# NoSuchThingAsRandom/EpidemicSimulator

Hardware: AMD Instinct MI355X
Metric: citizen-timesteps/sec (higher is better)
Workload: dtype u32 citizen word; u32 uniform vs ceil(q*2^32) (reference: f64 uniform; tolerance 2^-32 per draw); 1 GPU; uk64m: 64000000 citizens, 290000 Output Areas, 10 seeds, steps 1..667 of 5000, interventions on; seed=1592598545

## Files before the change

### epidemicsimulator_amd/csrc/esim_device.h

```cpp
#pragma once
#include <stdint.h>

#define CW_TE_SHIFT    19u
#define CW_BUS_EXPOSED (1u << 18)
#define CW_FLAGS       0xFFu
#define CW_VAX_SHIFT   11u
#define CW_VAX_MASK    (0x7Fu << CW_VAX_SHIFT)
#define CW_KEEP        (CW_FLAGS | CW_VAX_MASK)
#define CW_VAX_NONE    0xFFFFFFFFu
#define CW_PLAN_SKIP   (1u << 10)
#define CW_VAX_REL(w)  ((((w) >> CW_VAX_SHIFT) & 0x7Fu) ? 127u - (((w) >> CW_VAX_SHIFT) & 0x7Fu) : CW_VAX_NONE)
#define CW_VAX_FIELD(j) ((127u - (j)) << CW_VAX_SHIFT)
#define CW_TE(w)       ((w) >> CW_TE_SHIFT)
#define CW_MAKE(te, rest) (((te) << CW_TE_SHIFT) | (rest))
#define TE_SUSCEPTIBLE 0x1FFFu
#define TE_VACCINATED  0x1FFEu
#define TE_RECOVERED   0x1FFDu
#define TE_BIAS        512u
#define TE_SLOTS       8192u
#define ESIM_MAX_STEP  7600u

#define FL_USES_PT        0x01u
#define FL_MASK_COMPLIANT 0x02u
#define FL_SAME_AREA      0x04u
// ... 184 lines not shown
    uint32_t *prof_buf;
#endif
    uint32_t xf_n;
    const uint32_t *bld_area;
    uint32_t n_areas;
};

#define XA_HEADER 8u
#define XB_HEADER 8u
#define FREE_MAX 96u
#define HKEY_EMPTY 0xFFFFFFFFFFFFFFFFull
#define PLAN_W 4096u
#define XV_HEADER 8u
#define XS_CAP_MAX (1u << 20)
#define HOT_STRIDE 32u
#define SUBQ 64u
#define HOT_NEWEXP 0u
#define HOT_UNITS 64u
#define HOT_BIGPAIRS 128u
#define HOT_BIG 129u
#define HOT_PREV_NEWEXP 257u
#define HOT_RESET 257u
#define HOT_LOST 321u
#define HOT_COUNT 322u
#define RAISE(ctrl, code, where) do { (ctrl)->error = (uint32_t)(-(code)); (ctrl)->err_where = (where); } while (0)
enum { ERR_AT_BIG_LIST = 2, ERR_AT_ITEM_CHECK = 6, ERR_AT_ROUTE_ITEM = 7, ERR_AT_BIGPAIRS = 10, ERR_AT_SCHOOL = 11 };
#define UNIT_NOOP 0xFFFFFFFFu
#ifndef LOST_CAP
#define LOST_CAP 8192u
#endif
#define CHUNK_BUS_STEPS 32u
#define PAIR_K(per_wave, nbus) ((per_wave) * ((nbus) > 8u ? ((nbus) + 3u) / 4u : 2u))
#define COUNT_GRID 256u
#define EXP_ROWS 32u
#ifndef UNIT_INLINE
#define UNIT_INLINE 1024u
#endif
#ifndef UNIT_PAIRS
#define UNIT_PAIRS 1024u
#endif
#define CHUNK_ROUTE_MAX 2048u
```

### epidemicsimulator_amd/csrc/esim_host_ctx.h

```cpp
namespace {

thread_local std::string g_create_error;

struct Timing {
    bool phase = false, kernel = false;
    uint32_t stride = 16;
    hipEvent_t ev[5] = { nullptr, nullptr, nullptr, nullptr, nullptr };
    double phase_s[3] = { 0, 0, 0 };
    std::vector<hipEvent_t> kev; size_t kev_used = 0;
    hipEvent_t cev[2] = { nullptr, nullptr }; double chunk_ms = 0; uint64_t chunk_steps = 0, chunk_count = 0;
    std::vector<hipEvent_t> pkev; size_t pkev_used = 0; uint64_t pipe_steps = 0;
    hipEvent_t sev[2] = { nullptr, nullptr }; double small_ms = 0; uint64_t small_steps = 0;
    bool kdetail = false;
    std::vector<hipEvent_t> kdev; std::vector<int> kd_kind; size_t kd_used = 0;
    double kd_ms[ESIM_CK_N] = { 0 }; uint64_t kd_calls[ESIM_CK_N] = { 0 };
    bool host_trace = false;
    std::vector<std::pair<const char *, double>> ht;

    static void make_pair(hipEvent_t (&e)[2]) { if (!e[0]) { (void)hipEventCreate(&e[0]); (void)hipEventCreate(&e[1]); } }
    void clear()
    {
        phase_s[0] = phase_s[1] = phase_s[2] = 0;
        kev_used = 0; pkev_used = 0; pipe_steps = 0;
        small_ms = 0; small_steps = 0; chunk_ms = 0; chunk_steps = 0; chunk_count = 0;
// ... 61 lines not shown
    uint32_t step = 0;
    esim_params P;
    Ctrl h;
    uint32_t *words = nullptr, *hist = nullptr, *log_off = nullptr, *exp_step = nullptr;
    esim_step_result *records = nullptr;
    uint32_t *log = nullptr; size_t log_cap = 0;
    uint32_t last_chunk_pairs = 0; bool quiet = false, repair_armed = false, elig_seen = false;
    uint64_t vax_chunk_steps = 0, vax_chunk_cuts = 0, vax_chunk_repairs = 0;
};

struct Seam { uint32_t step = 0, rate = 0; uint64_t seed = 0; };

struct DrawSeam { uint32_t step = 0; bool twice = false, two_capacities = false; uint64_t seed = 0; double chance = 0.0, mask_effectiveness = 0.0; };

struct Tuning {
    uint32_t grid_citizens = 1, grid_infected = 1, grid_expose = 1;
    uint32_t grid_chunk = 1024;
    bool grid_chunk_env = false;
    bool pipeline = true;
    bool time_parallel = true;
    bool vax_chunks = true;
    bool vax_repair = true;
    bool vax_repair_always = false;
    uint32_t tiny_pairs = 2048;
    uint32_t small_grid = 64, small_mult = 4;
    uint32_t draw_mult = 4, units_mult = 4;
    uint32_t small_max = 128;
};

struct esim_ctx_impl {
    esim_params P;
    Dev d;
    bool uploaded = false;
    hipStream_t stream = nullptr;
    std::string err;
    std::vector<uint32_t> init_state;
    std::vector<uint32_t> init_log;
    size_t cnt_bytes = 0;
    uint32_t *cnt_base = nullptr;
    uint32_t n_routes = 0;
    size_t xa_n = 0, xb_n = 0, xf_n = 0;
    uint64_t pop_hash = 0;
    uint64_t pop_hash_head = 0;
    uint32_t cap_steps = 0;
    uint32_t *area_cnt = nullptr;
    uint32_t *arrival = nullptr;
// ... 243 lines not shown
```

### epidemicsimulator_amd/csrc/esim_host_run.h

```cpp
namespace {

int enqueue_begin(esim_ctx_impl *c, bool time_kernel)
{
    Dev &d = c->d;
    if (c->tm.phase) HIP_TRY(c, hipEventRecord(c->tm.ev[0], c->stream));
    if (time_kernel) HIP_TRY(c, hipEventRecord(c->tm.kev[c->tm.kev_used + 0], c->stream));
    hipLaunchKernelGGL(k_infected, dim3(c->tune.grid_infected), dim3(TPB), 0, c->stream, d);
    if (d.n_shards > 1) {
        const uint32_t n = (uint32_t)std::max<size_t>(XA_HEADER, std::max(d.n_shared_bld, d.n_shared_room));
        hipLaunchKernelGGL(k_pack_a, dim3(grid_for(n, TPB, 1u << 20)), dim3(TPB), 0, c->stream, d);
    }
    if (c->tm.phase) HIP_TRY(c, hipEventRecord(c->tm.ev[1], c->stream));
    return ESIM_OK;
}

int enqueue_exposures(esim_ctx_impl *c)
{
    Dev &d = c->d;
    if (d.n_shards > 1) {
        const uint32_t n = (uint32_t)std::max<size_t>(XA_HEADER, std::max(d.n_shared_bld, d.n_shared_room));
        hipLaunchKernelGGL(k_unpack_a, dim3(grid_for(n, TPB, 1u << 20)), dim3(TPB), 0, c->stream, d);
    }
    hipLaunchKernelGGL(k_expose, dim3(c->tune.grid_expose), dim3(TPB), 0, c->stream, d);
    if (d.n_shards > 1) hipLaunchKernelGGL(k_pack_b, dim3(VACC_WINDOW / TPB), dim3(TPB), 0, c->stream, d);
// ... 113 lines not shown
bool tiny_chunk(const esim_ctx_impl *c) { return c->tune.tiny_pairs && c->last_chunk_pairs <= c->tune.tiny_pairs && c->d.world == 1u && c->d.n_shards == 1u; }
bool small_chunk(const esim_ctx_impl *c) { return c->tune.small_grid && c->last_chunk_pairs < 4096u && c->tune.grid_chunk > c->tune.small_grid && !c->tune.grid_chunk_env; }

struct ChunkPass {
    esim_ctx_impl *c;
    uint32_t limit_t;
    bool kd;
    uint32_t n_ahead() const { return (uint32_t)c->xf_n; }
    void mark(int kind) const { if (kd) kd_mark(c, kind); }
    void future(uint32_t n) const { mark(ESIM_CK_FUTURE); hipLaunchKernelGGL(k_future, dim3(1), dim3(FIN_TPB), 0, c->stream, c->d, n, limit_t); }
    void decide(uint32_t n, int parallel, int vax_in_census) const { mark(ESIM_CK_DECIDE); hipLaunchKernelGGL(k_decide, dim3(1), dim3(64), 0, c->stream, c->d, n, limit_t, parallel, vax_in_census); }
    void vax_plan(int sharded) const { mark(ESIM_CK_VAX); hipLaunchKernelGGL(k_chunk_vax<false>, dim3(FREE_MAX + (sharded ? 0u : 1u)), dim3(FIN_TPB), 0, c->stream, c->d, n_ahead(), limit_t, sharded); }
    void lost() const { mark(ESIM_CK_VAX_REPAIR); hipLaunchKernelGGL(k_chunk_lost, dim3(1), dim3(FIN_TPB), 0, c->stream, c->d); }
    void vax_repair(int sharded) const { hipLaunchKernelGGL(k_chunk_vax<true>, dim3(FREE_MAX), dim3(FIN_TPB), 0, c->stream, c->d, n_ahead(), limit_t, sharded); }
    void front(bool few) const
    {
        const Tuning &t = c->tune;
        const uint32_t g = few ? t.small_grid : t.grid_chunk, g_draw = g * (few ? t.small_mult : t.draw_mult), g_units = g * (few ? t.small_mult : t.units_mult);
        mark(ESIM_CK_MARKS); hipLaunchKernelGGL(k_chunk_marks, dim3(g), dim3(TPB), 0, c->stream, c->d);
        mark(ESIM_CK_FOLD); hipLaunchKernelGGL(k_chunk_fold, dim3(g), dim3(TPB), 0, c->stream, c->d);
        mark(ESIM_CK_DRAW); hipLaunchKernelGGL(k_chunk_draw, dim3(g_draw), dim3(TPB), 0, c->stream, c->d, g * (TPB / 64u));
        mark(ESIM_CK_UNITS); hipLaunchKernelGGL(k_chunk_units, dim3(g_units), dim3(TPB), 0, c->stream, c->d);
    }
    void count() const { mark(ESIM_CK_COUNT); hipLaunchKernelGGL(k_chunk_count, dim3(COUNT_GRID), dim3(TPB), 0, c->stream, c->d); }
    void scatter() const { mark(ESIM_CK_SCATTER); hipLaunchKernelGGL(k_chunk_scatter, dim3(COUNT_GRID), dim3(TPB), 0, c->stream, c->d); }
    void books(int alone, int then_next) const { mark(ESIM_CK_BOOKS); hipLaunchKernelGGL(k_chunk_books, dim3(1), dim3(FIN_TPB), 0, c->stream, c->d, alone, then_next, n_ahead(), limit_t); }
    void vax_final() const { mark(ESIM_CK_VAX_FINAL); hipLaunchKernelGGL(k_chunk_vax_final, dim3(FREE_MAX), dim3(TPB), 0, c->stream, c->d); }
};

void enqueue_parallel_chunk(esim_ctx_impl *c, int then_next, uint32_t limit_t)
{
    const ChunkPass p{ c, limit_t, true };
    const bool alone = c->last_chunk_pairs < 1024u;
    p.front(small_chunk(c));
    if (!alone) p.count();
    p.books(alone ? 1 : 0, then_next);
    if (!alone) p.scatter();
    p.mark(ESIM_CK_N);
}

void enqueue_vax_chunk(esim_ctx_impl *c, uint32_t limit_t)
{
    const ChunkPass p{ c, limit_t, true };
    const Tuning &t = c->tune;
    const bool quiet = c->quiet && c->d.world == 1u;
    p.vax_plan(0);
    p.decide(p.n_ahead(), 1, 0);
    if (!quiet) {
        p.front(small_chunk(c));
        if (c->d.world == 1u && t.vax_repair && (c->repair_armed || t.vax_repair_always)) { p.lost(); p.vax_repair(0); }
    }
    p.count();
    p.books(0, 0);
    if (!quiet) p.scatter();
    p.vax_final();
    p.mark(ESIM_CK_N);
}

void enqueue_free_burst(esim_ctx_impl *c, uint32_t bursts, uint32_t limit_t)
{
    const ChunkPass p{ c, limit_t, true };
    if (tiny_chunk(c)) {
        for (uint32_t g = 0; g < bursts; ++g) {
            p.mark(ESIM_CK_TINY);
            hipLaunchKernelGGL(k_chunk_tiny, dim3(1), dim3(FIN_TPB), 0, c->stream, c->d, g == 0u ? 1 : 0, g + 1u < bursts ? 1 : 0, p.n_ahead(), limit_t);
        }
        p.mark(ESIM_CK_N);
        return;
    }
    p.future(p.n_ahead());
    p.decide(p.n_ahead(), 1, 0);
    for (uint32_t g = 0; g < bursts; ++g) enqueue_parallel_chunk(c, g + 1u < bursts ? 1 : 0, limit_t);
}

int run_chunk(esim_ctx_impl *c, uint32_t n_ahead, uint32_t *executed, Ctrl *state_before)
{
    Dev &d = c->d; Timing &t = c->tm;
// ... 233 lines not shown
```

### epidemicsimulator_amd/csrc/esim_host_shard.h

```cpp
namespace {

#define RCCL_ENTRIES(X) X(GetUniqueId) X(CommInitRank) X(CommDestroy) X(CommAbort) X(Send) X(Recv) X(GroupStart) X(GroupEnd) X(AllReduce) X(GetErrorString)
struct RcclApi {
#define X(f) decltype(&nccl##f) f = nullptr;
    RCCL_ENTRIES(X)
#undef X
    bool ok = false;
};

RcclApi &rccl()
{
    static RcclApi api;
    static bool tried = false;
    if (tried) return api;
    tried = true;
    void *h = nullptr;
    for (const char *name : { "librccl.so", "librccl.so.1" }) if ((h = dlopen(name, RTLD_NOW | RTLD_NOLOAD))) break;
    if (!h) for (const char *name : { "librccl.so.1", "librccl.so", "/opt/rocm/lib/librccl.so.1" }) if ((h = dlopen(name, RTLD_NOW | RTLD_GLOBAL))) break;
    if (!h) return api;
    api.ok = true;
#define X(f) if (!(api.f = (decltype(api.f))dlsym(h, "nccl" #f))) api.ok = false;
    RCCL_ENTRIES(X)
#undef X
    return api;
// ... 226 lines not shown
    int rc;
    p.future(n_ahead);
    if (vax) {
        hipLaunchKernelGGL(k_vax_live<false>, dim3(PLAN_W / TPB, FREE_MAX), dim3(TPB), 0, c->stream, d, n_ahead, limit_t);
        if ((rc = exchange_buf(c, 3, d.xv, xv_n))) return rc;
        p.vax_plan(1);
    }
    const size_t seg = 1u + 3u * (size_t)d.xs_cap;
    for (uint32_t r = 0; r < d.world; ++r) HIP_TRY(c, hipMemsetAsync(d.xs_out + (size_t)r * seg, 0, sizeof(uint32_t), c->stream));
    hipLaunchKernelGGL(k_shared_pack, dim3(256), dim3(TPB), 0, c->stream, d, n_ahead, limit_t);
    if ((rc = exchange_alltoall(c, 4, d.xs_out, d.xs, seg))) return rc;
    hipLaunchKernelGGL(k_shard_prep, dim3(1), dim3(128), 0, c->stream, d, n_ahead, limit_t);
    if ((rc = exchange(c, 2))) return rc;
    p.decide(n_ahead, 1, 1);
    p.front(false);
    if (vax && c->tune.vax_repair && (c->repair_armed || c->tune.vax_repair_always)) {
        p.lost();
        if ((rc = exchange_buf(c, 10, d.xl, FREE_MAX + 2u))) return rc;
        hipLaunchKernelGGL(k_lost_global, dim3(1), dim3(64), 0, c->stream, d);
        hipLaunchKernelGGL(k_vax_live<true>, dim3(PLAN_W / TPB, FREE_MAX), dim3(TPB), 0, c->stream, d, n_ahead, limit_t);
        if ((rc = exchange_buf(c, 3, d.xv, xv_n))) return rc;
        p.vax_repair(1);
    }
    p.count();
    if (vax && (rc = exchange_buf(c, 5, d.xc, FREE_MAX + 2u))) return rc;
    p.books(0, 0);
    p.scatter();
    p.vax_final();
    HIP_TRY(c, hipGetLastError());
    return ESIM_OK;
}

int run_coupled_steps(esim_ctx_impl *c, uint32_t n, bool ex)
{
    int rc;
    for (uint32_t s = 0; s < n; ++s) {
        const bool tk = want_kernel_timing(c);
        if ((rc = enqueue_begin(c, tk))) return rc;
        if (ex && (rc = exchange(c, 0))) return rc;
        if ((rc = enqueue_exposures(c))) return rc;
        if (ex && (rc = exchange(c, 1))) return rc;
        if ((rc = enqueue_finish(c, tk))) return rc;
        if ((s & 255u) == 255u && (rc = wait_stream(c))) return rc;
    }
    c->comm.step_steps += n;
    return ESIM_OK;
}

}

// ... 70 lines not shown
```

### epidemicsimulator_amd/csrc/esim_host_upload.h

```cpp
namespace {

struct UploadHost {
    const esim_population *pop;
    uint32_t N, B, R, n_global;
    bool sharded;
    std::vector<uint8_t> fl;
    std::vector<uint32_t> room_fixed;
    std::vector<uint32_t> route_off, riders, route_of;
    uint32_t n_routes = 0, max_route = 0, n_big_routes = 0;
    bool any_big = false;
    std::vector<uint32_t> res_off, res_idx, wrk_off, wrk_idx, room_off, room_idx;
    bool home_sorted = true;
};

int upload_validate(esim_ctx_impl *c, UploadHost &u)
{
    const esim_population *pop = u.pop; const uint32_t N = u.N, B = u.B, R = u.R;
    if (!pop->home_building || !pop->work_building || !pop->room || !pop->flags || !pop->building_area || !pop->building_type)
        return fail(c, ESIM_EINVAL, "esim_upload_population: a required array is NULL");
    if (R && !pop->room_building) return fail(c, ESIM_EINVAL, "esim_upload_population: room_building is NULL");
    if (pop->n_seeds && !pop->seeds) return fail(c, ESIM_EINVAL, "esim_upload_population: seeds is NULL");
    u.n_global = pop->n_citizens_global ? pop->n_citizens_global : N;
    if ((uint64_t)pop->citizen_id_base + N > u.n_global) return fail(c, ESIM_EINVAL, "esim_upload_population: shard range exceeds n_citizens_global");
    u.sharded = u.n_global != N || pop->n_shared_buildings || pop->n_shared_rooms;
// ... 184 lines not shown
        d.n_sch = n_sch;
        if ((rc = dev_upload(c, &d.sch_of_bld, sch_of.data(), sch_of.size()))) return rc;
    }
    {
        std::vector<uint4> w4(N ? N : 1);
        for (uint32_t i = 0; i < N; ++i) w4[i] = make_uint4(pop->home_building[i], pop->work_building[i], u.room_fixed[i], u.route_of[i]);
        if ((rc = dev_upload(c, &d.where4, w4.data(), w4.size()))) return rc;
        std::vector<BldRec> b8(B ? B : 1);
        for (uint32_t b = 0; b < B; ++b) b8[b] = BldRec{ u.res_off[b], u.res_off[b + 1], u.wrk_off[b], u.wrk_off[b + 1], (uint32_t)pop->building_type[b], ovf_off[b], ovf_off[b + 1], 0u };
        if ((rc = dev_upload(c, &d.bld8, b8.data(), b8.size()))) return rc;
        if ((rc = dev_alloc_fill(c, &d.sch_diff, (size_t)(d.n_sch ? d.n_sch : 1) * SD_REPL * 2u * FREE_MAX))) return rc;
    }
    d.ovf_room_base = ovf_off.back();
    d.ovf_n = d.ovf_room_base + u.room_off.back() + 1u;
    if ((rc = dev_alloc_fill(c, &d.ovf, (size_t)d.ovf_n))) return rc;
    d.n_wrk_idx = (uint32_t)u.wrk_idx.size(); d.n_room_idx = (uint32_t)u.room_idx.size();
    d.big_qcap = d.items_cap / SUBQ;
    if ((rc = dev_alloc_fill(c, &d.big_list, (size_t)d.big_qcap * SUBQ * 3u))) return rc;
    if ((rc = dev_alloc_fill(c, &d.used_pref, CHUNK_WAVES_MAX + 1u))) return rc;
    if ((rc = dev_alloc_fill(c, &d.pair_cnt, 16384u)) || (rc = dev_alloc_fill(c, &d.used_cnt, 16384u))) return rc;
    if ((rc = dev_alloc_fill(c, &d.hot, (size_t)HOT_COUNT * HOT_STRIDE))) return rc;
    d.newexp_cap = N / SUBQ + 1u;
    if ((rc = dev_alloc_fill(c, &d.newexp, (size_t)d.newexp_cap * SUBQ))) return rc;
    if ((rc = dev_alloc_fill(c, &d.cursor, (size_t)EXP_ROWS * FREE_MAX))) return rc;
    return ESIM_OK;
}

int upload_step_tables(esim_ctx_impl *c, const UploadHost &u)
{
    const uint32_t N = u.N, B = u.B, R = u.R;
    Dev &d = c->d; int rc;
    const size_t per_parity = (size_t)B + R + u.n_routes;
    for (int p = 0; p < (int)MARK_SLOTS; ++p) {
        uint32_t *base = c->cnt_base + p * per_parity;
        d.cnt_bld[p] = base; d.cnt_room[p] = base + B; d.route_flag[p] = base + B + R;
        if ((rc = dev_alloc(c, &d.touched_bld[p], B)) || (rc = dev_alloc(c, &d.touched_room[p], R))) return rc;
        if ((rc = dev_alloc(c, &d.touched_route[p], u.n_routes)) || (rc = dev_alloc(c, &d.touched_route_big[p], u.n_routes))) return rc;
    }
    if ((rc = dev_alloc(c, &d.vax_ev, (size_t)FREE_MAX * VACC_MAX_RATE))) return rc;
    if ((rc = dev_alloc_fill(c, &d.vax_cnt, FREE_MAX)) || (rc = dev_alloc_fill(c, &d.vax_now, FREE_MAX))) return rc;
    if ((rc = dev_alloc_fill(c, &d.vax_delta, 4u * (FREE_MAX + 2u)))) return rc;
    if ((rc = dev_alloc_fill(c, &d.lost_list, LOST_CAP))) return rc;
    if ((rc = dev_alloc_fill(c, &d.xf_adj, FREE_MAX + 2u))) return rc;
    if ((rc = dev_alloc(c, &d.hist, TE_SLOTS)) || (rc = dev_alloc(c, &d.log, (size_t)N + 1)) || (rc = dev_alloc(c, &d.log_off, TE_SLOTS + 1))) return rc;
    {
        const uint32_t *sd = nullptr;
        if ((rc = dev_upload(c, &sd, c->init_log.data(), c->init_log.size()))) return rc;
// ... 50 lines not shown
}

int upload_pinned(esim_ctx_impl *c, const UploadHost &u)
{
    if (!c->pin.ctrl) HIP_TRY(c, hipHostMalloc((void **)&c->pin.ctrl, sizeof(Ctrl), hipHostMallocDefault));
    if (!c->rs.stage) HIP_TRY(c, hipHostMalloc((void **)&c->rs.stage, sizeof(*c->rs.stage), hipHostMallocDefault));
    if (!c->rs.ev) HIP_TRY(c, hipEventCreateWithFlags(&c->rs.ev, hipEventDisableTiming));
    if (int rc = pinned_grow(c, &c->pin.rec, &c->pin.rec_n, (size_t)c->cap_steps + 1)) return rc;
    return pinned_grow(c, &c->pin.area, &c->pin.area_n, (size_t)u.pop->n_areas * 5u);
}

void upload_tuning(esim_ctx_impl *c, const UploadHost &u)
{
    Tuning &t = c->tune;
    t.grid_citizens = grid_for(u.N, TPB, 2048);
    t.grid_infected = 1024;
    t.grid_expose = 1024;
    if (const char *e = std::getenv("ESIM_GRID_INFECTED")) t.grid_infected = (uint32_t)std::max(1, std::atoi(e));
    const char *gc = std::getenv("ESIM_GRID_CHUNK");
    t.grid_chunk_env = gc != nullptr;
    if (gc) t.grid_chunk = (uint32_t)std::min((int)(CHUNK_WAVES_MAX * 64u / TPB), std::max(16, std::atoi(gc) / 16 * 16));
    if (std::getenv("ESIM_TRACE_HOST")) c->tm.host_trace = true;
    if (const char *e = std::getenv("ESIM_VAX_REPAIR")) { t.vax_repair = std::atoi(e) != 0; t.vax_repair_always = std::atoi(e) >= 2; }
    if (const char *e = std::getenv("ESIM_TINY_PAIRS")) t.tiny_pairs = (uint32_t)std::max(0, std::atoi(e));
    if (const char *e = std::getenv("ESIM_SMALL_GRID")) t.small_grid = (uint32_t)std::max(0, std::atoi(e) / 16 * 16);
    if (const char *e = std::getenv("ESIM_SMALL_MULT")) t.small_mult = (uint32_t)std::min(16, std::max(1, std::atoi(e)));
    if (const char *e = std::getenv("ESIM_DRAW_MULT")) t.draw_mult = (uint32_t)std::min(4, std::max(1, std::atoi(e)));
    if (const char *e = std::getenv("ESIM_UNITS_MULT")) t.units_mult = (uint32_t)std::min(16, std::max(1, std::atoi(e)));
    if (const char *e = std::getenv("ESIM_GRID_EXPOSE")) t.grid_expose = (uint32_t)std::max(1, std::atoi(e));
}

}

extern "C" int esim_upload_population(esim_ctx *ctx, const esim_population *pop)
{
    esim_ctx_impl *c = CTX(ctx);
    if (!c || !pop) return fail(c, ESIM_EINVAL, "esim_upload_population: null argument");
    HIP_TRY(c, hipSetDevice(c->P.device));
    UploadHost u;
    u.pop = pop; u.N = pop->n_citizens; u.B = pop->n_buildings; u.R = pop->n_rooms;
    int rc;
    if ((rc = upload_validate(c, u))) return rc;
    c->pop_hash = population_hash(pop, &c->pop_hash_head);
    upload_routes(u);
    upload_member_lists(u);
    c->init_state.resize(u.N);
// ... 164 lines not shown
```

### epidemicsimulator_amd/csrc/esim_kernels_books.h

```cpp
#pragma once
#include "esim_kernels_common.h"
#include "esim_kernels_plan.h"
#include "esim_kernels_marks.h"
__global__ __launch_bounds__(TPB) void k_chunk_count(Dev d)
{
    Ctrl *ctrl = d.ctrl;
    if (!ctrl->chunk_parallel || ctrl->chunk_ok == 0u) return;
    const uint32_t tid = blockIdx.x * TPB + threadIdx.x, r = tid & (SUBQ - 1u), step = (gridDim.x * TPB) / SUBQ;
    const uint32_t n_new = newexp_len(d, HOT_NEWEXP, r);
    const uint32_t *list = newexp_list(d, r);
    const uint32_t t0 = ctrl->chunk_t0;
    __shared__ uint32_t e_cnt[2u * FREE_MAX];
    __shared__ uint32_t s_cut;
    if (threadIdx.x < 2u * FREE_MAX) e_cnt[threadIdx.x] = 0u;
    if (threadIdx.x == 0) s_cut = 0xFFFFFFFFu;
    __syncthreads();
    for (uint32_t i = tid / SUBQ; i < n_new; i += step) {
        if (list[i] >= d.n) continue;
        const uint32_t w = d.cit[list[i]];
        const uint32_t j = CW_TE(w) - TE_BIAS - t0;
        if (j < FREE_MAX) atomicAdd(&e_cnt[2u * j + ((w & CW_BUS_EXPOSED) ? 1u : 0u)], 1u);
        if ((w & CW_BUS_EXPOSED) && CW_VAX_REL(w) != CW_VAX_NONE) { atomicMin(&s_cut, j); if (d.world > 1u) d.xc[j] = 1u; }
    }
    __syncthreads();
    if (threadIdx.x < 2u * FREE_MAX && e_cnt[threadIdx.x]) atomicAdd(&d.exp_part[(size_t)(blockIdx.x % EXP_ROWS) * 2u * FREE_MAX + threadIdx.x], e_cnt[threadIdx.x]);
    if (threadIdx.x == 0 && s_cut != 0xFFFFFFFFu) atomicMin(&ctrl->chunk_cut, s_cut);
    if (!ctrl->vax_chunk) return;
    __shared__ int dl[4][FREE_MAX + 2];
    for (uint32_t i = threadIdx.x; i < 4u * (FREE_MAX + 2u); i += TPB) (&dl[0][0])[i] = 0;
    __syncthreads();
    const uint32_t n = ctrl->chunk_ok;
    for (uint32_t j = blockIdx.x; j < n; j += gridDim.x) {
        const uint32_t cnt = d.vax_cnt[j];
        for (uint32_t i = threadIdx.x; i < cnt; i += TPB) {
            const uint32_t w = d.cit[d.vax_ev[(size_t)j * VACC_MAX_RATE + i]], te = CW_TE(w);
            if (CW_VAX_REL(w) != j) continue;
            atomicAdd(&dl[3][j + 1u], 1);
            if (te == TE_SUSCEPTIBLE || (te < TE_RECOVERED && te - TE_BIAS - t0 < n && te - TE_BIAS - t0 > j)) { atomicSub(&dl[0][j + 1u], 1); continue; }
            const int e_last = (int)te - (int)TE_BIAS + (int)d.exposed_time - (int)t0, i_last = e_last + 1 + (int)d.infected_time;
            const int lo = (int)j + 1;
            if (lo <= e_last) { atomicSub(&dl[1][lo], 1); atomicAdd(&dl[1][min(e_last, (int)n - 1) + 1], 1); }
            const int ilo = max(lo, e_last + 1);
            if (ilo <= i_last && ilo < (int)n) { atomicSub(&dl[2][ilo], 1); atomicAdd(&dl[2][min(i_last, (int)n - 1) + 1], 1); }
        }
    }
    __syncthreads();
    for (uint32_t i = threadIdx.x; i < 4u * (FREE_MAX + 2u); i += TPB) { const int v = (&dl[0][0])[i]; if (v) atomicAdd(&d.vax_delta[i], (uint32_t)v); }
}

__global__ __launch_bounds__(TPB) void k_chunk_scatter(Dev d)
{
    Ctrl *ctrl = d.ctrl;
    if (ctrl->chunk_done == 0u) return;
    const uint32_t t0 = ctrl->prev_t0;
    const uint32_t n_items = min(ctrl->prev_n_items, d.items_cap);
    {
        const uint32_t tid = blockIdx.x * TPB + threadIdx.x, r = tid & (SUBQ - 1u), step = (gridDim.x * TPB) / SUBQ;
        const uint32_t n_new = newexp_len(d, HOT_PREV_NEWEXP, r);
        const uint32_t *list = newexp_list(d, r);
        const uint32_t n_eff = ctrl->prev_n_eff;
        for (uint32_t i = tid / SUBQ; i < n_new; i += step) {
            const uint32_t m = list[i];
            if (m >= d.n) continue;
            const uint32_t te = CW_TE(d.cit[m]);
            if (te - TE_BIAS - t0 < n_eff) d.log[d.log_off[te] + atomicAdd(&d.cursor[(blockIdx.x % EXP_ROWS) * FREE_MAX + te - TE_BIAS - t0], 1u)] = m;
            else {
                const bool again = ctrl->prev_cut && te - TE_BIAS - t0 == n_eff && (d.cit[m] & CW_BUS_EXPOSED);
                atomicOr(&d.cit[m], (TE_SUSCEPTIBLE << CW_TE_SHIFT) | (again ? CW_PLAN_SKIP : 0u));
                atomicAnd(&d.cit[m], ~CW_BUS_EXPOSED);
            }
        }
    }
    const uint32_t per_wave = ctrl->prev_per_wave, n_mw = per_wave ? n_items / per_wave : 0u;
    const uint32_t tid = blockIdx.x * TPB + threadIdx.x, nth = gridDim.x * TPB;
    for (uint32_t i = tid; i < n_mw * per_wave; i += nth) {
        const uint32_t w = i / per_wave, k = i - w * per_wave;
        if (k >= d.used_cnt[w]) continue;
        const uint32_t h = d.hitems[i];
        if (h >= d.hcap) continue;
        const uint32_t state = d.slot_state[h];
        if (state > ITEM_RECS && d.item_rec[i].id < d.n_bld + d.n_room)
            for (uint32_t j = 0; j < FREE_MAX; ++j) d.vec[(size_t)h * FREE_MAX + j] = 0u;
        d.hkey[h] = HKEY_EMPTY;
        if (state) d.slot_state[h] = 0u;
    }
}

__global__ __launch_bounds__(TPB) void k_chunk_vax_final(Dev d)
{
    Ctrl *ctrl = d.ctrl;
    if (!ctrl->prev_vax) return;
    const uint32_t n_eff = ctrl->prev_n_eff;
    const uint32_t n = ctrl->prev_planned;
    for (uint32_t j = blockIdx.x; j < n; j += gridDim.x) {
        const uint32_t cnt = d.vax_cnt[j];
        for (uint32_t i = threadIdx.x; i < cnt; i += TPB) {
            const uint32_t c = d.vax_ev[(size_t)j * VACC_MAX_RATE + i];
            const uint32_t w = d.cit[c];
            if (CW_VAX_REL(w) != j) continue;
            if (j < n_eff) {
                const uint32_t te = CW_TE(w);
                if (te < TE_RECOVERED) atomicSub(&d.hist[te], 1u);
                d.cit[c] = CW_MAKE(TE_VACCINATED, w & (CW_BUS_EXPOSED | CW_FLAGS));
            } else atomicAnd(&d.cit[c], ~CW_VAX_MASK);
        }
    }
}

// ... 86 lines not shown
        ctrl->n_vaccinated = V0 + cum[3][n_eff];
        if (vax) ctrl->elig_count = elig0 - cum[4][n_eff];
        ctrl->log_len = run0 + (P[top0 + (int)n_eff] - P[top0]);
        ctrl->t = t0 + n_eff; ctrl->steps_done = t0 + n_eff - 1u;
        if (n_eff < n_cut) ctrl->finished = 1u;
        else if (n_cut < n) ctrl->vax_cuts += 1u;
        ctrl->prev_cut = (n_eff == n_cut && n_cut < n && !(vax && ctrl->repair_ran)) ? 1u : 0u;
        if (n_eff) {
            ctrl->lockdown = d.dec[n_eff].lockdown; ctrl->mask = d.dec[n_eff].mask;
            ctrl->at_work = d.dec[n_eff - 1u].at_work; ctrl->bus_dir = d.dec[n_eff - 1u].bus_dir;
        }
        const uint32_t keep = marks_left ? ((t0 + n - 1u) & (MARK_SLOTS - 1u)) : MARK_SLOTS;
        for (uint32_t z = 0; z < MARK_SLOTS; ++z)
            if (z != keep) { ctrl->n_touched_bld[z] = 0u; ctrl->n_touched_room[z] = 0u; ctrl->n_touched_route[z] = 0u; ctrl->n_touched_route_big[z] = 0u; }
    }
    return n_eff;
}

__global__ __launch_bounds__(FIN_TPB) void k_batch_finish(Dev d, uint32_t t0, uint32_t n)
{
    batch_finish_body(d, t0, n);
}

struct BooksShared { uint32_t e_cnt[2 * FREE_MAX]; uint32_t lo_s[FREE_MAX], cur_s[FREE_MAX]; uint32_t win[BF_WIN]; uint32_t wtmp[FIN_TPB / 64]; };
__device__ __forceinline__ void books_body(const Dev &d, int fused, int do_next, uint32_t max_ahead, uint32_t limit_t, BooksShared &bs)
{
    uint32_t *e_cnt = bs.e_cnt, *lo_s = bs.lo_s, *cur_s = bs.cur_s, *win = bs.win, *wtmp = bs.wtmp;
    Ctrl *ctrl = d.ctrl;
    const uint32_t tid = threadIdx.x;
    const uint32_t pb0 = PROF_NOW();
    if (!ctrl->chunk_parallel || ctrl->chunk_ok == 0u) {
        if (tid == 0) {
            ctrl->chunk_done = 0u;
            ctrl->prev_vax = ld(&ctrl->vax_chunk); ctrl->prev_n_eff = 0u; ctrl->prev_planned = ld(&ctrl->vax_planned); ctrl->vax_chunk = 0u;
        }
        return;
    }
    const uint32_t t0 = ctrl->chunk_t0, n = ctrl->chunk_ok;
    const uint32_t n_items = min(ld(&ctrl->n_items), d.items_cap);
    if (tid < 2u * FREE_MAX) e_cnt[tid] = 0u;
    if (tid < FREE_MAX) cur_s[tid] = 0u;
    __syncthreads();
    const uint32_t r = tid & (SUBQ - 1u);
    const uint32_t n_new = newexp_len(d, HOT_NEWEXP, r);
    const uint32_t *list = newexp_list(d, r);
    if (fused) {
        for (uint32_t i = tid / SUBQ; i < n_new; i += FIN_TPB / SUBQ) {
            if (list[i] >= d.n) continue;
            const uint32_t w = d.cit[list[i]];
            const uint32_t j = CW_TE(w) - TE_BIAS - t0;
            if (j < FREE_MAX) atomicAdd(&e_cnt[2u * j + ((w & CW_BUS_EXPOSED) ? 1u : 0u)], 1u);
        }
    } else if (tid < 2u * n) {
        uint32_t a = 0u, run = 0u;
        uint32_t v[EXP_ROWS];
#pragma unroll
        for (uint32_t p = 0; p < EXP_ROWS; ++p) v[p] = d.exp_part[(size_t)p * 2u * FREE_MAX + tid];
#pragma unroll
        for (uint32_t p = 0; p < EXP_ROWS; ++p) {
            d.exp_part[(size_t)p * 2u * FREE_MAX + tid] = 0u;
            a += v[p];
            if (!(tid & 1u)) d.cursor[p * FREE_MAX + (tid >> 1)] = run;
            run += v[p] + __shfl_xor(v[p], 1, 64);
        }
        e_cnt[tid] = a;
    }
    __syncthreads();
    const uint32_t pb1 = PROF_NOW();
    const bool vax = ld(&ctrl->vax_chunk) != 0u;
    const uint32_t n_eff = batch_finish_body(d, t0, n, e_cnt, lo_s, vax, false);
    const uint32_t pb2 = PROF_NOW();
    if (!fused) {
        if (tid < SUBQ) d.hot[(HOT_PREV_NEWEXP + tid) * HOT_STRIDE] = n_new;
        if (tid == 0) { ctrl->prev_t0 = t0; ctrl->prev_n_items = n_items; ctrl->prev_per_wave = ld(&ctrl->items_per_wave);
                        ctrl->prev_n = n; ctrl->prev_n_eff = n_eff; ctrl->prev_vax = vax ? 1u : 0u; ctrl->prev_planned = ld(&ctrl->vax_planned); ctrl->vax_chunk = 0u; }
    }
    if (tid == 0) ctrl->chunk_done = 1u;
    if (tid < 64u) {
        uint32_t a = ld(&d.hot[(HOT_NEWEXP + tid) * HOT_STRIDE]), b = ld(&d.hot[(HOT_UNITS + tid) * HOT_STRIDE]);
        for (int o = 32; o > 0; o >>= 1) { a += __shfl_xor(a, o, 64); b += __shfl_xor(b, o, 64); }
        if (tid == 0) { ctrl->n_newexp = a; ctrl->n_units = b; ctrl->n_route_pairs_big = ld(&d.hot[HOT_BIGPAIRS * HOT_STRIDE]); }
    }
    __syncthreads();
    if (fused) {
        for (uint32_t i = tid / SUBQ; i < n_new; i += FIN_TPB / SUBQ) {
            const uint32_t m = list[i];
            if (m >= d.n) continue;
            const uint32_t j = CW_TE(d.cit[m]) - TE_BIAS - t0;
            if (j < FREE_MAX) d.log[lo_s[j] + atomicAdd(&cur_s[j], 1u)] = m;
        }
        const uint32_t per_wave = ld(&ctrl->items_per_wave), n_mw = per_wave ? n_items / per_wave : 0u;
        for (uint32_t w0 = tid; w0 < n_mw; w0 += 4u * FIN_TPB) {
            uint32_t used[4], h[4][4];
#pragma unroll
            for (int a = 0; a < 4; ++a) { const uint32_t w = w0 + (uint32_t)a * FIN_TPB; used[a] = w < n_mw ? d.used_cnt[w] : 0u; }
#pragma unroll
            for (int a = 0; a < 4; ++a)
#pragma unroll
                for (int k = 0; k < 4; ++k) h[a][k] = (uint32_t)k < used[a] ? d.hitems[(w0 + (uint32_t)a * FIN_TPB) * per_wave + (uint32_t)k] : ITEM_UNUSED;
            uint32_t st[4][4];
#pragma unroll
            for (int a = 0; a < 4; ++a)
#pragma unroll
                for (int k = 0; k < 4; ++k) st[a][k] = h[a][k] < d.hcap ? d.slot_state[h[a][k]] : 0u;
#pragma unroll
            for (int a = 0; a < 4; ++a) {
                const uint32_t base = (w0 + (uint32_t)a * FIN_TPB) * per_wave;
// ... 7 lines not shown
                    if (state) d.slot_state[hs] = 0u;
                }
                for (uint32_t k = 4u; k < used[a]; ++k) {
                    const uint32_t hs = d.hitems[base + k];
                    if (hs >= d.hcap) continue;
                    const uint32_t state = d.slot_state[hs];
                    if (state > ITEM_RECS && d.item_rec[base + k].id < d.n_bld + d.n_room)
                        for (uint32_t j = 0; j < FREE_MAX; ++j) d.vec[(size_t)hs * FREE_MAX + j] = 0u;
                    d.hkey[hs] = HKEY_EMPTY;
                    if (state) d.slot_state[hs] = 0u;
                }
            }
        }
    }
    const uint32_t pb3 = PROF_NOW();
    if (do_next) {
        __syncthreads();
        future_body(d, max_ahead, limit_t, win, wtmp);
        __syncthreads();
        const uint32_t pb4 = PROF_NOW();
        if (tid < 64u) decide_body(d, max_ahead, limit_t, 1);
        BOOKS_PROF(d, 4, pb4 - pb3);
    }
    BOOKS_PROF(d, 0, pb1 - pb0); BOOKS_PROF(d, 1, pb2 - pb1); BOOKS_PROF(d, 2, pb3 - pb2); BOOKS_PROF(d, 3, PROF_NOW() - pb3);
    (void)pb0; (void)pb1; (void)pb2; (void)pb3;
}

__global__ __launch_bounds__(FIN_TPB) void k_chunk_books(Dev d, int fused, int do_next, uint32_t max_ahead, uint32_t limit_t)
{
    __shared__ BooksShared bs;
    books_body(d, fused, do_next, max_ahead, limit_t, bs);
}
```

Before: 57760 billion citizen-timesteps/s.

## Fuse chunk books and log scatter into one wide tail kernel

Adds a tail path, on by default when world==1, that moves hash-map cleanup into extra blocks of the count kernel. Books then runs as block 0 of a new multi-block tail kernel whose other blocks do the new-exposure log scatter for the current chunk, so the scatter no longer waits for the next chunk's scatter launch. Each block recomputes the prefix offsets from exp_part, and a last-block ticket zeroes exp_part. This removes a serial kernel launch and lets the single-block books work overlap the parallel scatter. In exchange it adds duplicated prefix work, ticket atomics and a second cursor array, and risks ordering bugs in the cut/skip logic.

```diff
diff --git a/epidemicsimulator_amd/csrc/esim_device.h b/epidemicsimulator_amd/csrc/esim_device.h
--- a/epidemicsimulator_amd/csrc/esim_device.h
+++ b/epidemicsimulator_amd/csrc/esim_device.h
@@ -230,7 +230,13 @@
 #define HOT_PREV_NEWEXP 257u
 #define HOT_RESET 257u
 #define HOT_LOST 321u
-#define HOT_COUNT 322u
+#define HOT_TAIL_RAN 322u
+#define HOT_TAIL_T0 323u
+#define HOT_TAIL_N 324u
+#define HOT_TAIL_VAX 325u
+#define HOT_TAIL_READERS 326u
+#define HOT_COUNT 327u
+#define HOT(d, i) ((d).hot[(i) * HOT_STRIDE])
 #define RAISE(ctrl, code, where) do { (ctrl)->error = (uint32_t)(-(code)); (ctrl)->err_where = (where); } while (0)
 enum { ERR_AT_BIG_LIST = 2, ERR_AT_ITEM_CHECK = 6, ERR_AT_ROUTE_ITEM = 7, ERR_AT_BIGPAIRS = 10, ERR_AT_SCHOOL = 11 };
 #define UNIT_NOOP 0xFFFFFFFFu
@@ -240,6 +246,7 @@
 #define CHUNK_BUS_STEPS 32u
 #define PAIR_K(per_wave, nbus) ((per_wave) * ((nbus) > 8u ? ((nbus) + 3u) / 4u : 2u))
 #define COUNT_GRID 256u
+#define CLEAN_GRID 1024u
 #define EXP_ROWS 32u
 #ifndef UNIT_INLINE
 #define UNIT_INLINE 1024u
diff --git a/epidemicsimulator_amd/csrc/esim_host_ctx.h b/epidemicsimulator_amd/csrc/esim_host_ctx.h
--- a/epidemicsimulator_amd/csrc/esim_host_ctx.h
+++ b/epidemicsimulator_amd/csrc/esim_host_ctx.h
@@ -107,6 +107,7 @@
     bool vax_chunks = true;
     bool vax_repair = true;
     bool vax_repair_always = false;
+    uint32_t chunk_tail = 2;
     uint32_t tiny_pairs = 2048;
     uint32_t small_grid = 64, small_mult = 4;
     uint32_t draw_mult = 4, units_mult = 4;
diff --git a/epidemicsimulator_amd/csrc/esim_host_run.h b/epidemicsimulator_amd/csrc/esim_host_run.h
--- a/epidemicsimulator_amd/csrc/esim_host_run.h
+++ b/epidemicsimulator_amd/csrc/esim_host_run.h
@@ -159,8 +159,15 @@
         mark(ESIM_CK_DRAW); hipLaunchKernelGGL(k_chunk_draw, dim3(g_draw), dim3(TPB), 0, c->stream, c->d, g * (TPB / 64u));
         mark(ESIM_CK_UNITS); hipLaunchKernelGGL(k_chunk_units, dim3(g_units), dim3(TPB), 0, c->stream, c->d);
     }
-    void count() const { mark(ESIM_CK_COUNT); hipLaunchKernelGGL(k_chunk_count, dim3(COUNT_GRID), dim3(TPB), 0, c->stream, c->d); }
-    void scatter() const { mark(ESIM_CK_SCATTER); hipLaunchKernelGGL(k_chunk_scatter, dim3(COUNT_GRID), dim3(TPB), 0, c->stream, c->d); }
+    void count(int tail) const { mark(ESIM_CK_COUNT); hipLaunchKernelGGL(k_chunk_count, dim3(COUNT_GRID + (tail ? CLEAN_GRID : 0u)), dim3(TPB), 0, c->stream, c->d, tail); }
+    void scatter(int clean) const { mark(ESIM_CK_SCATTER); hipLaunchKernelGGL(k_chunk_scatter, dim3(COUNT_GRID), dim3(TPB), 0, c->stream, c->d, clean); }
+    void tail(int then_next) const { mark(ESIM_CK_BOOKS); hipLaunchKernelGGL(k_chunk_tail, dim3(TAIL_GRID), dim3(FIN_TPB), 0, c->stream, c->d, then_next, n_ahead(), limit_t); }
+    void wide_tail(int then_next) const
+    {
+        const uint32_t form = c->d.world == 1u ? c->tune.chunk_tail : 0u;
+        if (form == 2u) { count(1); tail(then_next); }
+        else { count(form ? 1 : 0); books(0, then_next); scatter(form ? 0 : 1); }
+    }
     void books(int alone, int then_next) const { mark(ESIM_CK_BOOKS); hipLaunchKernelGGL(k_chunk_books, dim3(1), dim3(FIN_TPB), 0, c->stream, c->d, alone, then_next, n_ahead(), limit_t); }
     void vax_final() const { mark(ESIM_CK_VAX_FINAL); hipLaunchKernelGGL(k_chunk_vax_final, dim3(FREE_MAX), dim3(TPB), 0, c->stream, c->d); }
 };
@@ -170,9 +177,8 @@
     const ChunkPass p{ c, limit_t, true };
     const bool alone = c->last_chunk_pairs < 1024u;
     p.front(small_chunk(c));
-    if (!alone) p.count();
-    p.books(alone ? 1 : 0, then_next);
-    if (!alone) p.scatter();
+    if (alone) p.books(1, then_next);
+    else p.wide_tail(then_next);
     p.mark(ESIM_CK_N);
 }
 
@@ -187,9 +193,8 @@
         p.front(small_chunk(c));
         if (c->d.world == 1u && t.vax_repair && (c->repair_armed || t.vax_repair_always)) { p.lost(); p.vax_repair(0); }
     }
-    p.count();
-    p.books(0, 0);
-    if (!quiet) p.scatter();
+    if (quiet) { p.count(0); p.books(0, 0); }
+    else p.wide_tail(0);
     p.vax_final();
     p.mark(ESIM_CK_N);
 }
diff --git a/epidemicsimulator_amd/csrc/esim_host_shard.h b/epidemicsimulator_amd/csrc/esim_host_shard.h
--- a/epidemicsimulator_amd/csrc/esim_host_shard.h
+++ b/epidemicsimulator_amd/csrc/esim_host_shard.h
@@ -272,10 +272,10 @@
         if ((rc = exchange_buf(c, 3, d.xv, xv_n))) return rc;
         p.vax_repair(1);
     }
-    p.count();
+    p.count(0);
     if (vax && (rc = exchange_buf(c, 5, d.xc, FREE_MAX + 2u))) return rc;
     p.books(0, 0);
-    p.scatter();
+    p.scatter(1);
     p.vax_final();
     HIP_TRY(c, hipGetLastError());
     return ESIM_OK;
diff --git a/epidemicsimulator_amd/csrc/esim_host_upload.h b/epidemicsimulator_amd/csrc/esim_host_upload.h
--- a/epidemicsimulator_amd/csrc/esim_host_upload.h
+++ b/epidemicsimulator_amd/csrc/esim_host_upload.h
@@ -230,7 +230,7 @@
     if ((rc = dev_alloc_fill(c, &d.hot, (size_t)HOT_COUNT * HOT_STRIDE))) return rc;
     d.newexp_cap = N / SUBQ + 1u;
     if ((rc = dev_alloc_fill(c, &d.newexp, (size_t)d.newexp_cap * SUBQ))) return rc;
-    if ((rc = dev_alloc_fill(c, &d.cursor, (size_t)EXP_ROWS * FREE_MAX))) return rc;
+    if ((rc = dev_alloc_fill(c, &d.cursor, (size_t)2u * EXP_ROWS * FREE_MAX))) return rc;
     return ESIM_OK;
 }
 
@@ -327,6 +327,7 @@
     if (gc) t.grid_chunk = (uint32_t)std::min((int)(CHUNK_WAVES_MAX * 64u / TPB), std::max(16, std::atoi(gc) / 16 * 16));
     if (std::getenv("ESIM_TRACE_HOST")) c->tm.host_trace = true;
     if (const char *e = std::getenv("ESIM_VAX_REPAIR")) { t.vax_repair = std::atoi(e) != 0; t.vax_repair_always = std::atoi(e) >= 2; }
+    if (const char *e = std::getenv("ESIM_CHUNK_TAIL")) t.chunk_tail = (uint32_t)std::min(2, std::max(0, std::atoi(e)));
     if (const char *e = std::getenv("ESIM_TINY_PAIRS")) t.tiny_pairs = (uint32_t)std::max(0, std::atoi(e));
     if (const char *e = std::getenv("ESIM_SMALL_GRID")) t.small_grid = (uint32_t)std::max(0, std::atoi(e) / 16 * 16);
     if (const char *e = std::getenv("ESIM_SMALL_MULT")) t.small_mult = (uint32_t)std::min(16, std::max(1, std::atoi(e)));
diff --git a/epidemicsimulator_amd/csrc/esim_kernels_books.h b/epidemicsimulator_amd/csrc/esim_kernels_books.h
--- a/epidemicsimulator_amd/csrc/esim_kernels_books.h
+++ b/epidemicsimulator_amd/csrc/esim_kernels_books.h
@@ -2,14 +2,50 @@
 #include "esim_kernels_common.h"
 #include "esim_kernels_plan.h"
 #include "esim_kernels_marks.h"
-__global__ __launch_bounds__(TPB) void k_chunk_count(Dev d)
-{
-    Ctrl *ctrl = d.ctrl;
-    if (!ctrl->chunk_parallel || ctrl->chunk_ok == 0u) return;
-    const uint32_t tid = blockIdx.x * TPB + threadIdx.x, r = tid & (SUBQ - 1u), step = (gridDim.x * TPB) / SUBQ;
+__device__ __forceinline__ void map_cleanup(const Dev &d, uint32_t n_items, uint32_t per_wave, uint32_t gw, uint32_t n_gw, uint32_t lane)
+{
+    const uint32_t n_mw = per_wave ? n_items / per_wave : 0u;
+    for (uint32_t w = gw; w < n_mw; w += n_gw) {
+        const uint32_t used = min(d.used_cnt[w], per_wave), base = w * per_wave;
+        for (uint32_t k0 = lane; k0 < used; k0 += 4u * 64u) {
+            uint32_t h[4], st[4];
+#pragma unroll
+            for (uint32_t a = 0; a < 4u; ++a) h[a] = k0 + 64u * a < used ? d.hitems[base + k0 + 64u * a] : ITEM_UNUSED;
+#pragma unroll
+            for (uint32_t a = 0; a < 4u; ++a) st[a] = h[a] < d.hcap ? d.slot_state[h[a]] : 0u;
+#pragma unroll
+            for (uint32_t a = 0; a < 4u; ++a) {
+                if (h[a] >= d.hcap) continue;
+                if (st[a] > ITEM_RECS && d.item_rec[base + k0 + 64u * a].id < d.n_bld + d.n_room)
+                    for (uint32_t j = 0; j < FREE_MAX; ++j) d.vec[(size_t)h[a] * FREE_MAX + j] = 0u;
+                d.hkey[h[a]] = HKEY_EMPTY;
+                if (st[a]) d.slot_state[h[a]] = 0u;
+            }
+        }
+    }
+}
+
+__global__ __launch_bounds__(TPB) void k_chunk_count(Dev d, int tail)
+{
+    Ctrl *ctrl = d.ctrl;
+    const bool runs = ctrl->chunk_parallel && ctrl->chunk_ok != 0u;
+    if (tail && blockIdx.x == 0 && threadIdx.x == 0) {
+        HOT(d, HOT_TAIL_RAN) = runs ? 1u : 0u; HOT(d, HOT_TAIL_T0) = ctrl->chunk_t0; HOT(d, HOT_TAIL_N) = ctrl->chunk_ok; HOT(d, HOT_TAIL_VAX) = ctrl->vax_chunk;
+    }
+    if (!runs) return;
+    if (blockIdx.x >= COUNT_GRID) {
+        const uint32_t gt = (blockIdx.x - COUNT_GRID) * TPB + threadIdx.x;
+        map_cleanup(d, min(ctrl->n_items, d.items_cap), ctrl->items_per_wave, gt >> 6, ((gridDim.x - COUNT_GRID) * TPB) >> 6, gt & 63u);
+        return;
+    }
+    const uint32_t tid = blockIdx.x * TPB + threadIdx.x, r = tid & (SUBQ - 1u), step = (COUNT_GRID * TPB) / SUBQ;
     const uint32_t n_new = newexp_len(d, HOT_NEWEXP, r);
     const uint32_t *list = newexp_list(d, r);
     const uint32_t t0 = ctrl->chunk_t0;
+    if (tail) {
+        if (tid < SUBQ) d.hot[(HOT_PREV_NEWEXP + tid) * HOT_STRIDE] = n_new;
+        if (blockIdx.x < EXP_ROWS && threadIdx.x < FREE_MAX) d.cursor[(EXP_ROWS + blockIdx.x) * FREE_MAX + threadIdx.x] = 0u;
+    }
     __shared__ uint32_t e_cnt[2u * FREE_MAX];
     __shared__ uint32_t s_cut;
     if (threadIdx.x < 2u * FREE_MAX) e_cnt[threadIdx.x] = 0u;
@@ -30,7 +66,7 @@
     for (uint32_t i = threadIdx.x; i < 4u * (FREE_MAX + 2u); i += TPB) (&dl[0][0])[i] = 0;
     __syncthreads();
     const uint32_t n = ctrl->chunk_ok;
-    for (uint32_t j = blockIdx.x; j < n; j += gridDim.x) {
+    for (uint32_t j = blockIdx.x; j < n; j += COUNT_GRID) {
         const uint32_t cnt = d.vax_cnt[j];
         for (uint32_t i = threadIdx.x; i < cnt; i += TPB) {
             const uint32_t w = d.cit[d.vax_ev[(size_t)j * VACC_MAX_RATE + i]], te = CW_TE(w);
@@ -48,42 +84,31 @@
     for (uint32_t i = threadIdx.x; i < 4u * (FREE_MAX + 2u); i += TPB) { const int v = (&dl[0][0])[i]; if (v) atomicAdd(&d.vax_delta[i], (uint32_t)v); }
 }
 
-__global__ __launch_bounds__(TPB) void k_chunk_scatter(Dev d)
+__device__ __forceinline__ void log_scatter(const Dev &d, uint32_t tid, uint32_t t0, uint32_t n_eff, bool skip, const uint32_t *start, uint32_t *cur)
+{
+    const uint32_t r = tid & (SUBQ - 1u), step = (COUNT_GRID * TPB) / SUBQ, row = (tid / TPB) % EXP_ROWS;
+    const uint32_t n_new = newexp_len(d, HOT_PREV_NEWEXP, r);
+    const uint32_t *list = newexp_list(d, r);
+    for (uint32_t i = tid / SUBQ; i < n_new; i += step) {
+        const uint32_t m = list[i];
+        if (m >= d.n) continue;
+        const uint32_t w = d.cit[m], j = CW_TE(w) - TE_BIAS - t0;
+        if (j < n_eff) d.log[start[j] + atomicAdd(&cur[row * FREE_MAX + j], 1u)] = m;
+        else {
+            const bool again = skip && j == n_eff && (w & CW_BUS_EXPOSED);
+            atomicOr(&d.cit[m], (TE_SUSCEPTIBLE << CW_TE_SHIFT) | (again ? CW_PLAN_SKIP : 0u));
+            atomicAnd(&d.cit[m], ~CW_BUS_EXPOSED);
+        }
+    }
+}
+
+__global__ __launch_bounds__(TPB) void k_chunk_scatter(Dev d, int clean)
 {
     Ctrl *ctrl = d.ctrl;
     if (ctrl->chunk_done == 0u) return;
-    const uint32_t t0 = ctrl->prev_t0;
-    const uint32_t n_items = min(ctrl->prev_n_items, d.items_cap);
-    {
-        const uint32_t tid = blockIdx.x * TPB + threadIdx.x, r = tid & (SUBQ - 1u), step = (gridDim.x * TPB) / SUBQ;
-        const uint32_t n_new = newexp_len(d, HOT_PREV_NEWEXP, r);
-        const uint32_t *list = newexp_list(d, r);
-        const uint32_t n_eff = ctrl->prev_n_eff;
-        for (uint32_t i = tid / SUBQ; i < n_new; i += step) {
-            const uint32_t m = list[i];
-            if (m >= d.n) continue;
-            const uint32_t te = CW_TE(d.cit[m]);
-            if (te - TE_BIAS - t0 < n_eff) d.log[d.log_off[te] + atomicAdd(&d.cursor[(blockIdx.x % EXP_ROWS) * FREE_MAX + te - TE_BIAS - t0], 1u)] = m;
-            else {
-                const bool again = ctrl->prev_cut && te - TE_BIAS - t0 == n_eff && (d.cit[m] & CW_BUS_EXPOSED);
-                atomicOr(&d.cit[m], (TE_SUSCEPTIBLE << CW_TE_SHIFT) | (again ? CW_PLAN_SKIP : 0u));
-                atomicAnd(&d.cit[m], ~CW_BUS_EXPOSED);
-            }
-        }
-    }
-    const uint32_t per_wave = ctrl->prev_per_wave, n_mw = per_wave ? n_items / per_wave : 0u;
-    const uint32_t tid = blockIdx.x * TPB + threadIdx.x, nth = gridDim.x * TPB;
-    for (uint32_t i = tid; i < n_mw * per_wave; i += nth) {
-        const uint32_t w = i / per_wave, k = i - w * per_wave;
-        if (k >= d.used_cnt[w]) continue;
-        const uint32_t h = d.hitems[i];
-        if (h >= d.hcap) continue;
-        const uint32_t state = d.slot_state[h];
-        if (state > ITEM_RECS && d.item_rec[i].id < d.n_bld + d.n_room)
-            for (uint32_t j = 0; j < FREE_MAX; ++j) d.vec[(size_t)h * FREE_MAX + j] = 0u;
-        d.hkey[h] = HKEY_EMPTY;
-        if (state) d.slot_state[h] = 0u;
-    }
+    const uint32_t t0 = ctrl->prev_t0, tid = blockIdx.x * TPB + threadIdx.x;
+    log_scatter(d, tid, t0, ctrl->prev_n_eff, ctrl->prev_cut != 0u, d.log_off + TE_BIAS + t0, d.cursor);
+    if (clean) map_cleanup(d, min(ctrl->prev_n_items, d.items_cap), ctrl->prev_per_wave, tid >> 6, (gridDim.x * TPB) >> 6, tid & 63u);
 }
 
 __global__ __launch_bounds__(TPB) void k_chunk_vax_final(Dev d)
@@ -216,7 +241,18 @@
     batch_finish_body(d, t0, n);
 }
 
-struct BooksShared { uint32_t e_cnt[2 * FREE_MAX]; uint32_t lo_s[FREE_MAX], cur_s[FREE_MAX]; uint32_t win[BF_WIN]; uint32_t wtmp[FIN_TPB / 64]; };
+
+__device__ __forceinline__ uint32_t exp_part_ticket(const Dev &d) { return threadIdx.x == 0 ? atomicAdd(&HOT(d, HOT_TAIL_READERS), 1u) + 1u : 0u; }
+__device__ __forceinline__ void exp_part_zero_if_last(const Dev &d, uint32_t ticket, uint32_t *s_last)
+{
+    if (threadIdx.x == 0) *s_last = ticket == gridDim.x ? 1u : 0u;
+    __syncthreads();
+    if (!*s_last) return;
+    for (uint32_t i = threadIdx.x; i < EXP_ROWS * 2u * FREE_MAX; i += blockDim.x) d.exp_part[i] = 0u;
+    if (threadIdx.x == 0) HOT(d, HOT_TAIL_READERS) = 0u;
+}
+
+struct BooksShared { uint32_t e_cnt[2 * FREE_MAX]; uint32_t lo_s[FREE_MAX], cur_s[FREE_MAX]; uint32_t win[BF_WIN]; uint32_t wtmp[FIN_TPB / 64]; uint32_t last; };
 __device__ __forceinline__ void books_body(const Dev &d, int fused, int do_next, uint32_t max_ahead, uint32_t limit_t, BooksShared &bs)
 {
     uint32_t *e_cnt = bs.e_cnt, *lo_s = bs.lo_s, *cur_s = bs.cur_s, *win = bs.win, *wtmp = bs.wtmp;
@@ -238,7 +274,7 @@
     const uint32_t r = tid & (SUBQ - 1u);
     const uint32_t n_new = newexp_len(d, HOT_NEWEXP, r);
     const uint32_t *list = newexp_list(d, r);
-    if (fused) {
+    if (fused == 1) {
         for (uint32_t i = tid / SUBQ; i < n_new; i += FIN_TPB / SUBQ) {
             if (list[i] >= d.n) continue;
             const uint32_t w = d.cit[list[i]];
@@ -252,20 +288,21 @@
         for (uint32_t p = 0; p < EXP_ROWS; ++p) v[p] = d.exp_part[(size_t)p * 2u * FREE_MAX + tid];
 #pragma unroll
         for (uint32_t p = 0; p < EXP_ROWS; ++p) {
-            d.exp_part[(size_t)p * 2u * FREE_MAX + tid] = 0u;
+            if (fused == 0) d.exp_part[(size_t)p * 2u * FREE_MAX + tid] = 0u;
             a += v[p];
-            if (!(tid & 1u)) d.cursor[p * FREE_MAX + (tid >> 1)] = run;
+            if (fused == 0 && !(tid & 1u)) d.cursor[p * FREE_MAX + (tid >> 1)] = run;
             run += v[p] + __shfl_xor(v[p], 1, 64);
         }
         e_cnt[tid] = a;
     }
     __syncthreads();
+    const uint32_t ticket = fused == 2 ? exp_part_ticket(d) : 0u;
     const uint32_t pb1 = PROF_NOW();
     const bool vax = ld(&ctrl->vax_chunk) != 0u;
     const uint32_t n_eff = batch_finish_body(d, t0, n, e_cnt, lo_s, vax, false);
     const uint32_t pb2 = PROF_NOW();
-    if (!fused) {
-        if (tid < SUBQ) d.hot[(HOT_PREV_NEWEXP + tid) * HOT_STRIDE] = n_new;
+    if (fused != 1) {
+        if (fused == 0 && tid < SUBQ) d.hot[(HOT_PREV_NEWEXP + tid) * HOT_STRIDE] = n_new;
         if (tid == 0) { ctrl->prev_t0 = t0; ctrl->prev_n_items = n_items; ctrl->prev_per_wave = ld(&ctrl->items_per_wave);
                         ctrl->prev_n = n; ctrl->prev_n_eff = n_eff; ctrl->prev_vax = vax ? 1u : 0u; ctrl->prev_planned = ld(&ctrl->vax_planned); ctrl->vax_chunk = 0u; }
     }
@@ -276,7 +313,7 @@
         if (tid == 0) { ctrl->n_newexp = a; ctrl->n_units = b; ctrl->n_route_pairs_big = ld(&d.hot[HOT_BIGPAIRS * HOT_STRIDE]); }
     }
     __syncthreads();
-    if (fused) {
+    if (fused == 1) {
         for (uint32_t i = tid / SUBQ; i < n_new; i += FIN_TPB / SUBQ) {
             const uint32_t m = list[i];
             if (m >= d.n) continue;
@@ -330,6 +367,7 @@
         if (tid < 64u) decide_body(d, max_ahead, limit_t, 1);
         BOOKS_PROF(d, 4, pb4 - pb3);
     }
+    if (fused == 2) { __syncthreads(); exp_part_zero_if_last(d, ticket, &bs.last); }
     BOOKS_PROF(d, 0, pb1 - pb0); BOOKS_PROF(d, 1, pb2 - pb1); BOOKS_PROF(d, 2, pb3 - pb2); BOOKS_PROF(d, 3, PROF_NOW() - pb3);
     (void)pb0; (void)pb1; (void)pb2; (void)pb3;
 }
@@ -339,3 +377,52 @@
     __shared__ BooksShared bs;
     books_body(d, fused, do_next, max_ahead, limit_t, bs);
 }
+
+#define TAIL_GRID (1u + COUNT_GRID * TPB / FIN_TPB)
+__global__ __launch_bounds__(FIN_TPB) void k_chunk_tail(Dev d, int do_next, uint32_t max_ahead, uint32_t limit_t)
+{
+    __shared__ BooksShared bs;
+    if (blockIdx.x == 0) { books_body(d, 2, do_next, max_ahead, limit_t, bs); return; }
+    Ctrl *ctrl = d.ctrl;
+    if (HOT(d, HOT_TAIL_RAN) == 0u) return;
+    constexpr uint32_t ROWS_WG = FIN_TPB / TPB;
+    __shared__ uint32_t tot[2u * 64u], start[ROWS_WG][FREE_MAX];
+    const uint32_t tid = threadIdx.x, gtid = (blockIdx.x - 1u) * FIN_TPB + tid;
+    static_assert(EXP_ROWS % ROWS_WG == 0u && COUNT_GRID % ROWS_WG == 0u, "a workgroup's rows are consecutive");
+    const uint32_t t0 = HOT(d, HOT_TAIL_T0), n = HOT(d, HOT_TAIL_N), row0 = ((blockIdx.x - 1u) * ROWS_WG) % EXP_ROWS;
+    uint32_t off[ROWS_WG];
+    if (tid < 2u * FREE_MAX) {
+        uint32_t v[EXP_ROWS], run = 0u;
+#pragma unroll
+        for (uint32_t p = 0; p < EXP_ROWS; ++p) v[p] = d.exp_part[(size_t)p * 2u * FREE_MAX + tid];
+#pragma unroll
+        for (uint32_t p = 0; p < EXP_ROWS; ++p) {
+#pragma unroll
+            for (uint32_t q = 0; q < ROWS_WG; ++q) if (p == row0 + q) off[q] = run;
+            run += v[p] + __shfl_xor(v[p], 1, 64);
+        }
+        if (!(tid & 1u)) tot[tid >> 1] = run;
+    } else if (tid < 2u * 64u + FREE_MAX) tot[tid - FREE_MAX] = 0u;
+    __syncthreads();
+    const uint32_t ticket = exp_part_ticket(d);
+    if (tid < 64u) {
+        uint32_t v0 = tot[tid], v1 = tot[64u + tid];
+        const uint32_t own0 = v0, own1 = v1;
+        for (uint32_t o = 1; o < 64u; o <<= 1) { const uint32_t y0 = __shfl_up(v0, o, 64), y1 = __shfl_up(v1, o, 64); if (tid >= o) { v0 += y0; v1 += y1; } }
+        v1 += __shfl(v0, 63, 64);
+        const uint32_t run0 = d.log_off[t0 + TE_BIAS];
+        tot[tid] = run0 + v0 - own0; tot[64u + tid] = run0 + v1 - own1;
+    }
+    __syncthreads();
+    if (tid < 2u * FREE_MAX && !(tid & 1u)) {
+#pragma unroll
+        for (uint32_t q = 0; q < ROWS_WG; ++q) start[q][tid >> 1] = tot[tid >> 1] + off[q];
+    }
+    __syncthreads();
+    const bool vax = HOT(d, HOT_TAIL_VAX) != 0u;
+    const uint32_t n_cut = vax ? min(n, ctrl->chunk_cut) : n;
+    const bool skip = n_cut < n && !(vax && ctrl->repair_ran);
+    log_scatter(d, gtid, t0, n_cut, skip, start[tid / TPB], d.cursor + EXP_ROWS * FREE_MAX);
+    __syncthreads();
+    exp_part_zero_if_last(d, ticket, &bs.last);
+}
```

Result: slower. 56660 billion citizen-timesteps/s (-1.9%).
